# re-ovo/wgpu-path-tracing

Hardware: AMD Instinct MI355X
Metric: Msamples/s (rays x bounces / s) (higher is better)
Workload: dtype f32

## Files before the change

wgpu-path-tracing_amd/csrc/pipeline.hip:

```cpp
#include "pt_device.h"
#include "pt_math.h"

namespace {

constexpr int BLOCK = 256;

PT_DEV void camera_ray(const ptmi_camera &cam, uint32_t x, uint32_t y, uint32_t frame, v3 &org, v3 &dir,
                       uint32_t &rng) {
    rng = rng_seed(x, y, frame);
    float jx = rng_f(rng), jy = rng_f(rng);
    float px = (float)x + jx, py = (float)y + jy;
    float uvx = (px / (float)cam.width) * 2.0f - 1.0f;
    float uvy = (py / (float)cam.height) * 2.0f - 1.0f;
    float th = tan1(cam.fov * 0.5f);
    v3 fw = mk3(cam.forward[0], cam.forward[1], cam.forward[2]);
    v3 rt = mk3(cam.right[0], cam.right[1], cam.right[2]);
    v3 up = mk3(cam.up[0], cam.up[1], cam.up[2]);
    v3 pos = mk3(cam.position[0], cam.position[1], cam.position[2]);
    v3 a = scale3(scale3(scale3(rt, uvx), th), cam.aspect);
    v3 b = scale3(scale3(up, uvy), th);
    dir = normalize3(add3(add3(fw, a), b));
    org = pos;
    if (cam.aperture > 0.0f) {
        v3 focal = madd3(dir, cam.focus_distance, pos);
// ... 39 lines not shown
#define PT_TILE_WORDS 1024
#endif
constexpr int TILE_WORDS = PT_TILE_WORDS;
constexpr int TILE_WAVES = TILE_WORDS / 64;

__global__ __launch_bounds__(TILE_WORDS) void k_tile_sums(const uint32_t *__restrict__ count_ptr,
                                                          const uint64_t *__restrict__ alive,
                                                          const uint64_t *__restrict__ shadow,
                                                          uint32_t *__restrict__ tile_sums,
                                                          uint32_t *__restrict__ shadow_tile_sums,
                                                          unsigned long long *__restrict__ stats, uint32_t bounce) {
    __shared__ uint32_t wsum[TILE_WAVES], wssum[TILE_WAVES];
    const uint32_t count = *count_ptr;
    const uint32_t nwords = (count + 63u) >> 6;
    if (blockIdx.x == 0 && threadIdx.x == 0) {
        atomicAdd(&stats[0], (unsigned long long)count); atomicAdd(&stats[8 + bounce], (unsigned long long)count);
    }
    if (blockIdx.x * TILE_WORDS >= nwords) return;
    const uint32_t w = blockIdx.x * TILE_WORDS + threadIdx.x;
    uint32_t c = 0, sc = 0;
    if (w < nwords) { c = (uint32_t)__popcll(alive[w]); if (shadow) sc = (uint32_t)__popcll(shadow[w]); }
    for (int off = 32; off > 0; off >>= 1) { c += __shfl_down(c, off); sc += __shfl_down(sc, off); }
    if ((threadIdx.x & 63u) == 0u) { wsum[threadIdx.x >> 6] = c; wssum[threadIdx.x >> 6] = sc; }
    __syncthreads();
    if (threadIdx.x == 0) {
        uint32_t t = 0, ts = 0;
        for (int i = 0; i < TILE_WAVES; i++) { t += wsum[i]; ts += wssum[i]; }
        tile_sums[blockIdx.x] = t;
        shadow_tile_sums[blockIdx.x] = ts;
        if (ts) { atomicAdd(&stats[1], (unsigned long long)ts); atomicAdd(&stats[2], (unsigned long long)ts); }
    }
}

PT_DEV void scatter_tile(uint32_t tile, const uint32_t *__restrict__ count_ptr, const uint32_t *__restrict__ queue,
                         const uint64_t *__restrict__ alive, const uint32_t *__restrict__ tile_sums,
                         uint32_t *__restrict__ next_queue, uint32_t *__restrict__ next_count) {
    __shared__ uint32_t wtot[TILE_WAVES];
    __shared__ uint32_t tile_base;
    const uint32_t count = *count_ptr;
    const uint32_t nwords = (count + 63u) >> 6;
    const uint32_t ntiles = (nwords + TILE_WORDS - 1) / TILE_WORDS;
    if (tile >= ntiles) {
        if (ntiles == 0 && tile == 0 && threadIdx.x == 0) *next_count = 0;
        return;
    }
    const uint32_t lane = threadIdx.x & 63u, wave = threadIdx.x >> 6;
    uint32_t pre = 0;
    for (uint32_t t = threadIdx.x; t < tile; t += TILE_WORDS) pre += tile_sums[t];
    for (int off = 32; off > 0; off >>= 1) pre += __shfl_down(pre, off);
    if (lane == 0) wtot[wave] = pre;
    __syncthreads();
    if (threadIdx.x == 0) { uint32_t t = 0; for (int i = 0; i < TILE_WAVES; i++) t += wtot[i]; tile_base = t; }
    __syncthreads();
    const uint32_t base0 = tile_base;
    __syncthreads();
    const uint32_t w = tile * TILE_WORDS + threadIdx.x;
    const uint64_t m = w < nwords ? alive[w] : 0ull;
    const uint32_t c = (uint32_t)__popcll(m);
    uint32_t inc = c;
    for (int off = 1; off < 64; off <<= 1) { uint32_t v = __shfl_up(inc, off); if (lane >= (uint32_t)off) inc += v; }
    if (lane == 63u) wtot[wave] = inc;
    __syncthreads();
    uint32_t wbase = 0;
    for (uint32_t i = 0; i < wave; i++) wbase += wtot[i];
    const uint32_t my_off = base0 + wbase + inc - c;
    if (tile == ntiles - 1 && threadIdx.x == TILE_WORDS - 1) *next_count = my_off + c;
    const uint32_t mlo = (uint32_t)m, mhi = (uint32_t)(m >> 32);
    const uint32_t w0 = tile * TILE_WORDS + wave * 64u;
    for (uint32_t j = 0; j < 64u; j++) {
        const uint32_t jlo = __shfl(mlo, (int)j), jhi = __shfl(mhi, (int)j), jbase = __shfl(my_off, (int)j);
        const uint64_t jm = ((uint64_t)jhi << 32) | jlo;
        if (jm == 0ull) continue;
        if ((jm >> lane) & 1ull) {
            const uint32_t below = (uint32_t)__popcll(jm & ((1ull << lane) - 1ull));
            const uint32_t slot = (w0 + j) * 64u + lane;
            next_queue[jbase + below] = queue ? queue[slot] : slot;
        }
    }
}

__global__ __launch_bounds__(TILE_WORDS) void k_scatter(const uint32_t *__restrict__ count_ptr,
                                                        const uint32_t *__restrict__ queue,
                                                        const uint64_t *__restrict__ alive,
                                                        const uint32_t *__restrict__ tile_sums,
                                                        uint32_t *__restrict__ next_queue,
                                                        uint32_t *__restrict__ next_count) {
    scatter_tile(blockIdx.x, count_ptr, queue, alive, tile_sums, next_queue, next_count);
}
__global__ __launch_bounds__(TILE_WORDS) void k_scatter2(uint32_t tiles, const uint32_t *__restrict__ count_ptr,
                                                         const uint32_t *__restrict__ queue,
                                                         const uint64_t *__restrict__ alive, const uint64_t *__restrict__ shadow,
                                                         const uint32_t *__restrict__ tile_sums, const uint32_t *__restrict__ shadow_sums,
                                                         uint32_t *__restrict__ next_queue, uint32_t *__restrict__ next_count,
                                                         uint32_t *__restrict__ shadow_queue, uint32_t *__restrict__ shadow_count) {
    if (blockIdx.x < tiles) scatter_tile(blockIdx.x, count_ptr, queue, alive, tile_sums, next_queue, next_count);
    else scatter_tile(blockIdx.x - tiles, count_ptr, nullptr, shadow, shadow_sums, shadow_queue, shadow_count);
}

__global__ __launch_bounds__(BLOCK) void k_accumulate(DevBand band, uint32_t frame0, uint32_t n_frames,
                                                      const float *__restrict__ L, uint32_t l_stride, float4 *__restrict__ out) {
    const uint32_t npix = band.rows * band.width;
    for (uint32_t pix = blockIdx.x * BLOCK + threadIdx.x; pix < npix; pix += gridDim.x * BLOCK) {
        const size_t oi = (size_t)band.row_of(pix / band.width) * band.width + pix % band.width;
        float4 acc = out[oi];
        for (uint32_t k = 0; k < n_frames; k++) {
            const size_t li = (size_t)k * npix + pix;
            rgb_sc l;
            if (l_stride == 4u) { const float4 v = reinterpret_cast<const float4 *>(L)[li]; l = rgb_sc{v.x, v.y, v.z}; }
            else l = reinterpret_cast<const rgb_sc *>(L)[li];
            float cx = min1(l.x, 2.5f), cy = min1(l.y, 2.5f), cz = min1(l.z, 2.5f);
            uint32_t frame = frame0 + k;
            if (frame > 0u) {
                float t = 1.0f / (float)(frame + 1u);
                cx = mix1(acc.x, cx, t); cy = mix1(acc.y, cy, t); cz = mix1(acc.z, cz, t);
            }
            acc = make_float4(cx, cy, cz, 0.0f);
        }
        out[oi] = acc;
    }
}

__global__ __launch_bounds__(BLOCK) void k_accumulate_aov(DevBand band, uint32_t frame0, uint32_t n_frames, const float4 *__restrict__ rec,
                                                          const ptmi_triangle *__restrict__ tris, uint32_t n_tris,
                                                          float4 *__restrict__ albedo, float4 *__restrict__ normal, uint2 *__restrict__ ids) {
    const uint32_t npix = band.rows * band.width;
    for (uint32_t pix = blockIdx.x * BLOCK + threadIdx.x; pix < npix; pix += gridDim.x * BLOCK) {
        const size_t oi = (size_t)band.row_of(pix / band.width) * band.width + pix % band.width;
        float4 a = albedo ? albedo[oi] : make_float4(0.0f, 0.0f, 0.0f, 0.0f);
        float4 n = normal ? normal[oi] : make_float4(0.0f, 0.0f, 0.0f, 0.0f);
// ... 136 lines not shown
}

}

void pt_launch_exact_math(hipStream_t s, int which, unsigned long long *out) {
    hipLaunchKernelGGL(k_exact_math, dim3(256 * 16), dim3(256), 0, s, which, out);
}
void pt_launch_raygen(hipStream_t s, int blocks, const ptmi_camera &cam, DevBand band, uint32_t frame0,
                      uint32_t n_frames, DevPaths p, uint32_t *count_out) {
    hipLaunchKernelGGL(k_raygen, dim3(blocks), dim3(BLOCK), 0, s, cam, band, frame0, n_frames, p, count_out);
}
void pt_launch_raygen_list(hipStream_t s, const ptmi_camera &cam, uint32_t n, const uint32_t *xs,
                           const uint32_t *ys, const uint32_t *frames, DevPaths p) {
    hipLaunchKernelGGL(k_raygen_list, dim3((n + BLOCK - 1) / BLOCK), dim3(BLOCK), 0, s, cam, n, xs, ys, frames, p);
}
void pt_launch_compact(hipStream_t s, int tiles, const uint32_t *queue, const uint32_t *count,
                       const uint64_t *alive_mask, const uint64_t *shadow_mask, uint32_t *tile_sums,
                       uint32_t *next_queue, uint32_t *next_count, uint32_t *shadow_queue, uint32_t *shadow_count,
                       unsigned long long *stats, uint32_t bounce, int do_scatter) {
    uint32_t *shadow_sums = tile_sums + tiles;
    hipLaunchKernelGGL(k_tile_sums, dim3(tiles), dim3(TILE_WORDS), 0, s, count, alive_mask, shadow_mask, tile_sums,
                       shadow_sums, stats, bounce);
#ifndef PT_NO_SCATTER2
    if (do_scatter && shadow_mask) {
        hipLaunchKernelGGL(k_scatter2, dim3(2 * tiles), dim3(TILE_WORDS), 0, s, (uint32_t)tiles, count, queue, alive_mask, shadow_mask,
                           tile_sums, shadow_sums, next_queue, next_count, shadow_queue, shadow_count);
        return;
    }
#endif
    if (do_scatter)
        hipLaunchKernelGGL(k_scatter, dim3(tiles), dim3(TILE_WORDS), 0, s, count, queue, alive_mask, tile_sums,
                           next_queue, next_count);
    if (shadow_mask)
        hipLaunchKernelGGL(k_scatter, dim3(tiles), dim3(TILE_WORDS), 0, s, count, (const uint32_t *)nullptr,
                           shadow_mask, shadow_sums, shadow_queue, shadow_count);
}
void pt_launch_accumulate(hipStream_t s, int blocks, DevBand band, uint32_t frame0, uint32_t n_frames,
                          const float *L, uint32_t l_stride, float4 *out) {
    hipLaunchKernelGGL(k_accumulate, dim3(blocks), dim3(BLOCK), 0, s, band, frame0, n_frames, L, l_stride, out);
}
void pt_launch_accumulate_aov(hipStream_t s, int blocks, DevBand band, uint32_t frame0, uint32_t n_frames, const float4 *rec,
                              const ptmi_triangle *tris, uint32_t n_tris, float4 *albedo, float4 *normal, uint2 *ids) {
    hipLaunchKernelGGL(k_accumulate_aov, dim3(blocks), dim3(BLOCK), 0, s, band, frame0, n_frames, rec, tris, n_tris, albedo, normal,
                       ids);
}
void pt_launch_accumulate_moments(hipStream_t s, int blocks, DevBand band, uint32_t frame0, uint32_t n_frames, const float *L,
                                  uint32_t l_stride, float4 *mom) {
    hipLaunchKernelGGL(k_accumulate_moments, dim3(blocks), dim3(BLOCK), 0, s, band, frame0, n_frames, L, l_stride, mom);
}
void pt_launch_pack_rows(hipStream_t s, int blocks, DevBand band, const float4 *frame, float4 *packed) {
    hipLaunchKernelGGL(k_pack_rows, dim3(blocks), dim3(BLOCK), 0, s, band, frame, packed);
}
void pt_launch_unpack_rows(hipStream_t s, int blocks, DevBand band, const float4 *packed, float4 *frame) {
    hipLaunchKernelGGL(k_unpack_rows, dim3(blocks), dim3(BLOCK), 0, s, band, packed, frame);
}
void pt_launch_blit(hipStream_t s, int blocks, uint32_t W, uint32_t H, const float4 *color, float4 *out_f32,
                    uint32_t *out_rgba8) {
    hipLaunchKernelGGL(k_blit, dim3(blocks), dim3(BLOCK), 0, s, W, H, color, out_f32, out_rgba8);
}
void pt_launch_math(hipStream_t s, int op, uint32_t n, const float *a, const float *b, const float *c, float *out) {
    hipLaunchKernelGGL(k_math, dim3((n + 255) / 256), dim3(256), 0, s, op, n, a, b, c, out);
}

uint32_t pt_compact_tile_slots(void) { return TILE_WORDS * 64u; }
```

wgpu-path-tracing_amd/csrc/pt_device.h:

```cpp
#pragma once
#include <hip/hip_runtime.h>
#include <stdint.h>
#include "ptmi_layout.h"

#define PT_HD __host__ __device__ inline

#define PT_REF_LEAF      0x80000000u
#define PT_REF_NONE      0xFFFFFFFFu
#define PT_LEAF_MAX_TRIS 32u
#define PT_LEAF_OFF_BITS 26u
#define PT_LEAF_OFF_MASK ((1u << PT_LEAF_OFF_BITS) - 1u)

struct DevScene;
struct DevScene {
    const ptmi_triangle *tris;  uint32_t n_tris;
    const ptmi_material *mats;  uint32_t n_mats;
    const ptmi_light *lights;   uint32_t n_lights;
    const void *atlas;          uint32_t atlas_w, atlas_h, atlas_fmt;
    const float4 *wnodes;       uint32_t n_wnodes;
    const float4 *tripos;
    float root_min[3], root_max[3];
    uint32_t root_ref;
    const float4 *ref_wnodes;   uint32_t ref_root_ref, has_fast;
    const uint4 *qnodes;        const uint32_t *leaf_stream;
// ... 4 lines not shown
    const float4 *ref_tripos;
    const float4 *tri_leafbox;
    float ref_root_min[3], ref_root_max[3];
    float safe_origin;
    const float4 *wnodes16, *ref_wnodes16;
    uint32_t root_ref16, ref_root_ref16;
    const uint4 *qnodes16;
    unsigned long long *verify_stat;
    const DevScene *self;
};

struct rgb_sc { float x, y, z; };
struct DevPaths {
    float4 *O, *D; float2 *C; float *L; uint32_t l_stride = 3;
    __device__ __forceinline__ rgb_sc ldL(uint32_t p) const {
        if (l_stride == 4u) { const float4 v = reinterpret_cast<const float4 *>(L)[p]; return rgb_sc{v.x, v.y, v.z}; }
        return reinterpret_cast<const rgb_sc *>(L)[p];
    }
    __device__ __forceinline__ void stL(uint32_t p, float x, float y, float z) const {
        if (l_stride == 4u) reinterpret_cast<float4 *>(L)[p] = make_float4(x, y, z, 0.0f);
        else reinterpret_cast<rgb_sc *>(L)[p] = rgb_sc{x, y, z};
    }
};
struct DevShadow { float4 *SO, *SD; rgb_sc *SC; uint32_t cap; };

struct DevBand {
    uint32_t width, height, y0, y1, strip, parts, part, rows;
    PT_HD uint32_t row_of(uint32_t l) const {
        if (parts <= 1u) return y0 + l;
        return y0 + ((l / strip) * parts + part) * strip + l % strip;
    }
};

struct ShadeParams {
    uint32_t bounce, max_bounces, do_mis;
    unsigned long long *stats;
    uint32_t emit_records;
};

enum { PT_VARIANT_GLOBAL = 1, PT_VARIANT_LDS = 2, PT_VARIANT_LDS_NODES = 3,
       PT_VARIANT_OWN_LDS = 4, PT_VARIANT_OWN_LDS_NODES = 5, PT_VARIANT_OWN_QLDS = 6, PT_VARIANT_OWN_QLDS_NODES = 7,
       PT_VARIANT_OWN_QGLOBAL = 8, PT_VARIANT_OWN_GLOBAL = 9,
       PT_VARIANT_OWN_LDS16_NODES = 10,
       PT_VARIANT_OWN_QLDS16_NODES = 11,
       PT_VARIANT_COUNT };

enum PtNodes {
    PT_NODES_EXACT,
    PT_NODES_QUANT,
    PT_NODES_EXACT16,
    PT_NODES_QUANT16 };
enum PtWhere {
    PT_LDS_ALL,
    PT_LDS_NODES,
    PT_FROM_MEMORY };
enum PtStack {
    PT_STACK_DEPTH,
    PT_STACK_NODES,
    PT_STACK_SPILL,
    PT_STACK_16BIT,
    PT_STACK_16BIT_SPILL };
struct PtVariant { PtNodes nodes; PtWhere where; PtStack stack; bool own; };
constexpr PtVariant kPtVariants[PT_VARIANT_COUNT] = {
    {},
    {PT_NODES_EXACT,   PT_FROM_MEMORY, PT_STACK_SPILL,       false},
    {PT_NODES_EXACT,   PT_LDS_ALL,     PT_STACK_DEPTH,       false},
    {PT_NODES_EXACT,   PT_LDS_NODES,   PT_STACK_NODES,       false},
    {PT_NODES_EXACT,   PT_LDS_ALL,     PT_STACK_DEPTH,       true},
    {PT_NODES_EXACT,   PT_LDS_NODES,   PT_STACK_NODES,       true},
    {PT_NODES_QUANT,   PT_LDS_ALL,     PT_STACK_DEPTH,       true},
// ... 22 lines not shown
    int wgs_per_cu;
    size_t lds_bytes;
    uint32_t *spill;
    int wants_spill;
    int quantized;
};
inline uint32_t pt_variant_code(const TraverseConfig &cfg) { return (uint32_t)cfg.variant * 10u + (uint32_t)cfg.wgs_per_cu; }
#ifndef PT_QCACHE_NODES
#define PT_QCACHE_NODES 256
#endif
#define PT_SPILL_ENTRIES 64
size_t pt_spill_bytes(int blocks);

void pt_launch_raygen(hipStream_t s, int blocks, const ptmi_camera &cam, DevBand band, uint32_t frame0,
                      uint32_t n_frames, DevPaths p, uint32_t *count_out);
void pt_launch_raygen_list(hipStream_t s, const ptmi_camera &cam, uint32_t n, const uint32_t *xs,
                           const uint32_t *ys, const uint32_t *frames, DevPaths p);
void pt_launch_extend(hipStream_t s, int blocks, const TraverseConfig &cfg, const DevScene &sc, DevPaths p,
                      const uint32_t *queue, const uint32_t *count, float2 *hits);
void pt_launch_extend_own(hipStream_t s, int blocks, const TraverseConfig &cfg, const DevScene &sc, DevPaths p,
                          const uint32_t *queue, const uint32_t *count, float2 *hits);
void pt_launch_hit_uv(hipStream_t s, uint32_t n, const DevScene &sc, DevPaths p, const float2 *hits, float2 *uv);
void pt_launch_shadow(hipStream_t s, int blocks, const TraverseConfig &cfg, const DevScene &sc, DevPaths p,
                      DevShadow sh, const uint32_t *shadow_queue, const uint32_t *count, uint8_t *occluded_out);
void pt_launch_shadow_own(hipStream_t s, int blocks, const TraverseConfig &cfg, const DevScene &sc, DevPaths p,
                          DevShadow sh, const uint32_t *shadow_queue, const uint32_t *count, uint8_t *occluded_out);
void pt_launch_shade(hipStream_t s, int blocks, const DevScene &sc, DevPaths p, const uint32_t *queue,
                     const uint32_t *count, const float2 *hits, DevShadow sh, uint64_t *alive_mask,
                     uint64_t *shadow_mask, ShadeParams sp, float4 *aov = nullptr);
void pt_launch_shade_fast(hipStream_t s, int blocks, const DevScene &sc, DevPaths p, const uint32_t *queue,
                          const uint32_t *count, const float2 *hits, DevShadow sh, uint64_t *alive_mask,
                          uint64_t *shadow_mask, ShadeParams sp, float4 *aov = nullptr);
uint32_t pt_compact_tile_slots(void);
void pt_launch_compact(hipStream_t s, int tiles, const uint32_t *queue, const uint32_t *count,
                       const uint64_t *alive_mask, const uint64_t *shadow_mask, uint32_t *tile_sums,
                       uint32_t *next_queue, uint32_t *next_count, uint32_t *shadow_queue, uint32_t *shadow_count,
                       unsigned long long *stats, uint32_t bounce, int do_scatter);
void pt_launch_accumulate(hipStream_t s, int blocks, DevBand band, uint32_t frame0, uint32_t n_frames,
                          const float *L, uint32_t l_stride, float4 *out);
void pt_launch_accumulate_aov(hipStream_t s, int blocks, DevBand band, uint32_t frame0, uint32_t n_frames, const float4 *rec,
                              const ptmi_triangle *tris, uint32_t n_tris, float4 *albedo, float4 *normal, uint2 *ids);
void pt_launch_accumulate_moments(hipStream_t s, int blocks, DevBand band, uint32_t frame0, uint32_t n_frames, const float *L,
                                  uint32_t l_stride, float4 *mom);
struct DenoiseArgs {
    uint32_t W, H, iterations;
    float phi_color, phi_normal, phi_depth;
};
void pt_launch_denoise(hipStream_t s, const DenoiseArgs &a, const float4 *radiance, const float4 *normal, const float4 *albedo,
                       const float4 *moments, float4 *guide, float *grad, float4 *cv, float4 *tmp, float4 *out);
void pt_launch_blit(hipStream_t s, int blocks, uint32_t W, uint32_t H, const float4 *color, float4 *out_f32,
                    uint32_t *out_rgba8);
void pt_launch_pack_rows(hipStream_t s, int blocks, DevBand band, const float4 *frame, float4 *packed);
void pt_launch_unpack_rows(hipStream_t s, int blocks, DevBand band, const float4 *packed, float4 *frame);
struct ptmi_options;
DevBand pt_band_of(const ptmi_options &opt, uint32_t width, uint32_t height);
struct ptmi_ctx;
struct PtPrepared;
PtPrepared *pt_prepare_scene(ptmi_ctx *c, const ptmi_triangle *tris, uint32_t nt, const ptmi_material *mats, uint32_t nm,
                             const ptmi_bvh_node *nodes, uint32_t nn, const ptmi_light *lights, uint32_t nl, int *rc_out);
int pt_install_scene(ptmi_ctx *c, PtPrepared *p);
void pt_free_prepared(PtPrepared *p);
int pt_atlas_bytes(uint32_t width, uint32_t height, int format, size_t *bytes, char *why, size_t why_len);
hipStream_t pt_ctx_stream(ptmi_ctx *c);
float4 *pt_ctx_output(ptmi_ctx *c);
int pt_ctx_device(const ptmi_ctx *c);
int pt_ctx_cus(const ptmi_ctx *c);
// ... 4 lines not shown
```

wgpu-path-tracing_amd/csrc/ptmi_api.hip:

```cpp
#include "ptmi.h"
#include "pt_device.h"
#include "fast_tree.h"

#include <algorithm>
#include <chrono>
#include <cmath>
#include <cstdarg>
#include <cstdint>
#include <cstdio>
#include <cstring>
#include <deque>
#include <memory>
#include <string>
#include <typeinfo>
#include <utility>
#include <vector>

namespace {

thread_local std::string g_create_err;

enum SceneBuf {
    kTris, kMats, kLights,
    kRefWnodes, kRefTripos,
    kWnodes, kTripos,
    kQnodes, kLeafStream,
    kLeafbox,
    kWnodes16, kRefWnodes16, kQnodes16,
    kSceneBufs
};

struct EventPair { hipEvent_t a, b; int kind; };
constexpr size_t kMaxPendingEvents = 4096;

}

struct Lane {
    size_t cap = 0;
    DevPaths paths{};
    float2 *hits = nullptr;
    DevShadow sh[2]{};
    uint32_t *queue[2] = {nullptr, nullptr}, *sq[2] = {nullptr, nullptr};
    uint64_t *alive = nullptr, *shadowm = nullptr;
    size_t mask_words = 0;
    uint32_t *word_off = nullptr, *counts = nullptr;
    uint32_t *d_spill = nullptr;
    uint32_t *d_spill_side = nullptr;
    uint8_t *d_occ = nullptr;
    hipStream_t side = nullptr;
    hipEvent_t ev_ready = nullptr, ev_shadow[2] = {nullptr, nullptr};
    float4 *aov = nullptr;
};

struct ptmi_ctx {
    int device = 0, n_cu = 256;
    hipStream_t own_stream = nullptr, stream = nullptr;
    Lane lane;
    mutable std::string err;
    bool alloc_oom = false;
    ptmi_options opt{};

    void *buf[kSceneBufs] = {};
    void *d_atlas = nullptr;
    DevScene *d_scene = nullptr;
    DevScene sc{};
    bool have_scene = false;
    ptmi_image_info img{};

    uint32_t W = 0, H = 0;
    float4 *d_out_own = nullptr, *d_out = nullptr;
    uint32_t aov_mask = 0;
    float4 *d_aov_albedo = nullptr, *d_aov_normal = nullptr;
    uint2 *d_aov_id = nullptr;
    bool moments_on = false;
    float4 *d_moments = nullptr;
// ... 74 lines not shown
constexpr size_t kMaxDispatchesInFlight = 256;

hipError_t throttle(ptmi_ctx *c, size_t max) {
    while (!c->in_flight.empty() && hipEventQuery(c->in_flight.front()) == hipSuccess) {
        c->event_pool.push_back(c->in_flight.front()); c->in_flight.pop_front();
    }
    (void)hipGetLastError();
    while (c->in_flight.size() > max) {
        hipError_t e = hipEventSynchronize(c->in_flight.front());
        if (e != hipSuccess) return e;
        c->event_pool.push_back(c->in_flight.front()); c->in_flight.pop_front();
    }
    return hipSuccess;
}

struct Timed {
    ptmi_ctx *c; hipEvent_t a = nullptr, b = nullptr; int kind; bool on;
    hipStream_t st;
    Timed(ptmi_ctx *c_, int kind_, bool on_, hipStream_t st_ = nullptr) : c(c_), kind(kind_), on(on_), st(st_ ? st_ : c_->stream) {
        if (on) { a = get_event(c); b = get_event(c); (void)hipEventRecord(a, st); }
    }
    ~Timed() {
        if (!on) return;
        (void)hipEventRecord(b, st);
        c->pending.push_back({a, b, kind});
        if (c->pending.size() > kMaxPendingEvents) drain_completed_events(c);
    }
};

void free_batch(Lane &ln) {
    dfree(ln.paths.O); dfree(ln.paths.D); dfree(ln.paths.C); dfree(ln.paths.L);
    dfree(ln.hits);
    for (int k = 0; k < 2; k++) { dfree(ln.sh[k].SO); ln.sh[k].SD = nullptr; ln.sh[k].SC = nullptr; dfree(ln.sq[k]); }
    dfree(ln.queue[0]); dfree(ln.queue[1]); dfree(ln.alive); dfree(ln.shadowm); dfree(ln.word_off); dfree(ln.d_occ);
    dfree(ln.aov);
    ln.cap = 0;
}

hipError_t sync_all(ptmi_ctx *c) {
    hipError_t e = c->stream ? hipStreamSynchronize(c->stream) : hipSuccess;
    if (e == hipSuccess && c->lane.side) e = hipStreamSynchronize(c->lane.side);
    if (e == hipSuccess && c->stream) e = hipStreamSynchronize(c->stream);
    return e;
}

constexpr size_t kBytesPerPath = 16 + 16 + 8 + 16 + 8 + 2 * (16 + 16 + sizeof(rgb_sc) + 4) + 2 * 4 + 1 + 1;
constexpr size_t kAovBytesPerPath = 32;
size_t bytes_per_path(bool aov) { return kBytesPerPath + (aov ? kAovBytesPerPath : 0); }

int ensure_capacity(ptmi_ctx *c, Lane &ln, size_t n) {
    const bool aov = c->aov_mask != 0;
    if (n <= ln.cap && (!aov || ln.aov)) return PTMI_OK;
    HIP_TRY(c, sync_all(c));
    free_batch(ln);
    size_t cap = (n + 1023) & ~(size_t)1023;
    size_t words = cap / 64 + 1;
    size_t tiles = cap / pt_compact_tile_slots() + 2;
    c->alloc_oom = false;
#define ALLOC(ptr, bytes) do { hipError_t e_ = hipMalloc(&(ptr), (bytes)); if (e_ != hipSuccess) { \
        c->alloc_oom = e_ == hipErrorOutOfMemory; free_batch(ln); (void)hipGetLastError(); \
        return fail(c, PTMI_E_HIP, "hipMalloc of %zu bytes for a batch of %zu paths failed: %s", (size_t)(bytes), cap, hipGetErrorString(e_)); } } while (0)
    ALLOC(ln.paths.O, cap * 16); ALLOC(ln.paths.D, cap * 16);
    ALLOC(ln.paths.C, cap * 8); ALLOC(ln.paths.L, cap * 16);
    ALLOC(ln.hits, cap * 8);
    for (int k = 0; k < 2; k++) {
        ALLOC(ln.sh[k].SO, cap * (16 + 16 + sizeof(rgb_sc)));
        ln.sh[k].SD = ln.sh[k].SO + cap; ln.sh[k].SC = reinterpret_cast<rgb_sc *>(ln.sh[k].SO + 2 * cap); ln.sh[k].cap = (uint32_t)cap;
        ALLOC(ln.sq[k], cap * 4);
    }
    ALLOC(ln.queue[0], cap * 4); ALLOC(ln.queue[1], cap * 4);
    ALLOC(ln.alive, words * 8); ALLOC(ln.shadowm, words * 8); ln.mask_words = words;
    ALLOC(ln.word_off, 2 * tiles * 4);
    ALLOC(ln.d_occ, cap);
    if (aov) ALLOC(ln.aov, cap * kAovBytesPerPath);
#undef ALLOC
    ln.cap = cap;
    return PTMI_OK;
}

struct HeldBuf {
    bool present = false;
    std::shared_ptr<const void> keep;
    const std::type_info *type = nullptr;
    const void *host = nullptr;
    void *dev = nullptr;
    int device = -1;
    size_t bytes = 0;
};

struct Built {
    HeldBuf buf[kSceneBufs];
    ptmi_image_info img{};
    uint32_t ref_root_ref = PT_REF_NONE;
    float ref_root_min[3] = {0, 0, 0}, ref_root_max[3] = {0, 0, 0};
    uint32_t root_ref16 = PT_REF_NONE, ref_root_ref16 = PT_REF_NONE;
    uint32_t q_top = 0;
    float tri_safe_dsum = 0.0f;
    uint32_t tree_builder_used = 0;
    double tree_ms = 0.0;

    Built() { img.leaves_used = 1; img.root_ref = PT_REF_NONE; }
    Built(const Built &) = delete;
// ... 732 lines not shown
    const TraverseConfig cfg0 = traverse_config(c, true), cfg_shadow0 = traverse_config(c, false);
    if (c->opt.traversal == PTMI_TRAVERSAL_LDS && pt_variant(cfg0.variant).where != PT_LDS_ALL)
        return fail(c, PTMI_E_UNSUPPORTED, "scene needs %zu B of LDS plus the stack; it does not fit in %zu B", lds_scene_bytes(c), kLdsMax);
    for (;;) {
        rc = ensure_capacity(c, ln, (size_t)(npix * F));
        if (rc == PTMI_OK) break;
        if (!auto_F || !c->alloc_oom || F <= 1) return rc;
        F = (F + 1) / 2;
    }
    if (cfg0.wants_spill && !ln.d_spill) HIP_TRY(c, hipMalloc(&ln.d_spill, pt_spill_bytes(c->n_cu * 8)));
    if (cfg_shadow0.wants_spill && !ln.d_spill_side) HIP_TRY(c, hipMalloc(&ln.d_spill_side, pt_spill_bytes(c->n_cu * 8)));
    c->st.traversal_used = pt_variant(cfg0.variant).where == PT_FROM_MEMORY ? PTMI_TRAVERSAL_GLOBAL : PTMI_TRAVERSAL_LDS;
    c->st.extend_variant = pt_variant_code(cfg0);
    c->st.shadow_variant = pt_variant_code(cfg_shadow0);
    c->st.frames_per_batch_used = F;
    c->st.radiance_stride_bytes = (walks_memory_quantised(cfg0) || walks_memory_quantised(cfg_shadow0)) ? 16u : 12u;
    const int blocks = c->n_cu * 8;
#ifndef PT_SHADE_WGS_PER_CU
#define PT_SHADE_WGS_PER_CU 16
#endif
    const int shade_blocks = c->n_cu * PT_SHADE_WGS_PER_CU;
    const uint32_t maxb = c->opt.max_bounces;
    const bool t1 = c->opt.timing >= 1, t2 = c->opt.timing >= 2, t3 = c->opt.timing >= 3;
    {
        Timed td(c, 0, t1);
        const hipStream_t ms = c->stream;
        const hipStream_t ss = side ? ln.side : ms;
        const int tiles = (int)(ln.cap / pt_compact_tile_slots() + 1);
        TraverseConfig cfg = cfg0, cfg_shadow = cfg_shadow0;
        cfg.spill = ln.d_spill; cfg_shadow.spill = side ? ln.d_spill_side : ln.d_spill;
        if (cfg_shadow.wants_spill && !cfg_shadow.spill) cfg_shadow.spill = ln.d_spill_side;
        ln.paths.l_stride = c->st.radiance_stride_bytes / 4u;
        const DevPaths bp = ln.paths;
        float4 *const aov_rec = c->aov_mask ? ln.aov : nullptr;
        for (uint32_t f0 = 0; f0 < n_frames; f0 += F) {
            const uint32_t fb = std::min(F, n_frames - f0);
            const uint32_t frame0 = cam->frame_index + f0;
            { Timed t(c, 4, t3, ms); pt_launch_raygen(ms, blocks, *cam, band, frame0, fb, bp, &ln.counts[0]); }
            int cur = 0;
            for (uint32_t b = 0; b < maxb; b++) {
                const uint32_t *q = b == 0 ? nullptr : ln.queue[cur];
                const int par = side ? (int)(b & 1u) : 0;
                const ShadeParams shp{b, maxb, c->opt.do_mis, c->d_stats, side ? 1u : 0u};
                { Timed t(c, 1, t2, ms); (c->sc.own ? pt_launch_extend_own : pt_launch_extend)(ms, blocks, cfg, c->sc, bp, q, &ln.counts[b], ln.hits); }
                const bool last = b + 1 == maxb;
                if (side && b >= 2) HIP_TRY(c, hipStreamWaitEvent(ms, ln.ev_shadow[par], 0));
                { Timed t(c, 2, t3, ms);
                  (c->opt.perf_mode ? pt_launch_shade_fast : pt_launch_shade)(
                      ms, shade_blocks, c->sc, bp, q, &ln.counts[b], ln.hits, ln.sh[par], ln.alive, ln.shadowm, shp,
                      b == 0 ? aov_rec : nullptr); }
                { Timed t(c, 5, t3, ms);
                  pt_launch_compact(ms, tiles, q, &ln.counts[b], ln.alive, nee ? ln.shadowm : nullptr,
                                    ln.word_off, ln.queue[cur ^ 1], &ln.counts[b + 1], ln.sq[par], &ln.counts[kShadowCount + par],
                                    c->d_stats, b, last ? 0 : 1); }
                if (side) {
                    HIP_TRY(c, hipEventRecord(ln.ev_ready, ms));
                    HIP_TRY(c, hipStreamWaitEvent(ss, ln.ev_ready, 0));
                    { Timed t(c, 3, t3, ss);
                      (c->sc.own ? pt_launch_shadow_own : pt_launch_shadow)(ss, blocks, cfg_shadow, c->sc, bp, ln.sh[par], ln.sq[par],
                                                                            &ln.counts[kShadowCount + par], nullptr); }
                    HIP_TRY(c, hipEventRecord(ln.ev_shadow[par], ss));
                } else if (nee) {
                    Timed t(c, 3, t3, ms);
                    (c->sc.own ? pt_launch_shadow_own : pt_launch_shadow)(ms, blocks, cfg_shadow, c->sc, bp, ln.sh[0], ln.sq[0], &ln.counts[kShadowCount], nullptr);
                }
                cur ^= 1;
            }
            if (side) {
                HIP_TRY(c, hipStreamWaitEvent(ms, ln.ev_shadow[(maxb - 1) & 1u], 0));
                if (maxb >= 2) HIP_TRY(c, hipStreamWaitEvent(ms, ln.ev_shadow[maxb & 1u], 0));
            }
            { Timed t(c, 6, t3, ms);
              pt_launch_accumulate(ms, blocks, band, frame0, fb, bp.L, bp.l_stride, c->d_out);
              if (aov_rec)
                  pt_launch_accumulate_aov(ms, blocks, band, frame0, fb, aov_rec, c->sc.tris, c->sc.n_tris, c->d_aov_albedo,
                                           c->d_aov_normal, c->d_aov_id);
              if (c->d_moments) pt_launch_accumulate_moments(ms, blocks, band, frame0, fb, bp.L, bp.l_stride, c->d_moments); }
        }
    }
    HIP_TRY(c, hipGetLastError());
    {
        hipEvent_t done = get_event(c);
        HIP_TRY(c, hipEventRecord(done, c->stream));
        c->in_flight.push_back(done);
        if (c->in_flight.size() > kMaxDispatchesInFlight) HIP_TRY(c, throttle(c, kMaxDispatchesInFlight));
    }
    c->st.paths += npix * n_frames;
// ... 492 lines not shown
```

wgpu-path-tracing_amd/csrc/shade.hip:

```cpp
#include "pt_device.h"
#include "pt_math.h"

namespace {

struct HitInfo {
    v3 position; float t;
    v3 normal;
    v3 albedo;
    float roughness, metallic, transmission, ior;
    v3 emission; float emissive_strength;
    bool is_front;
};

PT_DEV v3 ld3(const float *p) { return mk3(p[0], p[1], p[2]); }

PT_DEV v4 atlas_load(const DevScene &sc, uint32_t x, uint32_t y) {
    v4 r; r.x = r.y = r.z = r.w = 0.0f;
    if (sc.atlas_fmt == 0u || x >= sc.atlas_w || y >= sc.atlas_h) return r;
    size_t idx = ((size_t)y * sc.atlas_w + x);
    if (sc.atlas_fmt == 1u) {
        const uint2 raw = reinterpret_cast<const uint2 *>(sc.atlas)[idx];
        union { uint32_t u; _Float16 h[2]; } a, b;
        a.u = raw.x; b.u = raw.y;
        r.x = (float)a.h[0]; r.y = (float)a.h[1]; r.z = (float)b.h[0]; r.w = (float)b.h[1];
// ... 209 lines not shown
        v3 to_l = sub3(lp, hit_pos);
        float dist = length3(to_l);
        v3 wi = vdiv3(to_l, dist);
        v3 e1 = sub3(ld3(T.v1), ld3(T.v0)), e2 = sub3(ld3(T.v2), ld3(T.v0));
        float area = length3(cross3(e1, e2)) * 0.5f;
        float cos_t = __builtin_fabsf(dot3(n, neg3(wi)));
        ls.pdf = (inv_n * rcp1(area)) * (dist * dist / max1(cos_t, PT_EPS));
        ls.intensity = scale3(ld3(lt.color), lt.intensity);
        ls.wi = wi;
        ls.dist = dist;
        ls.traced = true;
    }
    return ls;
}

constexpr int SBLOCK = 256;
#ifndef PT_SHADE_WAVES
#define PT_SHADE_WAVES 0
#endif
#if PT_SHADE_WAVES > 0
#define PT_SHADE_ATTR __attribute__((amdgpu_waves_per_eu(PT_SHADE_WAVES)))
#else
#define PT_SHADE_ATTR
#endif

template <bool AOV>
__global__ __launch_bounds__(SBLOCK) PT_SHADE_ATTR void k_shade(DevScene sc, DevPaths P, const uint32_t *__restrict__ queue,
                                                  const uint32_t *__restrict__ count_ptr,
                                                  const float2 *__restrict__ hits, DevShadow S,
                                                  uint64_t *__restrict__ alive_mask,
                                                  uint64_t *__restrict__ shadow_mask, ShadeParams sp,
                                                  float4 *__restrict__ aov) {
    const uint32_t count = *count_ptr;
    uint32_t n_skipped = 0, n_emitted = 0;
    for (uint32_t base = blockIdx.x * SBLOCK; base < count; base += gridDim.x * SBLOCK) {
        const uint32_t i = base + threadIdx.x;
        bool alive = false, shadow = false, skipped = false, emitted = false;
        if (i < count) {
            const uint32_t q = queue ? queue[i] : i;
            const float2 h2 = ld_stream(&hits[i]);
            if (!(h2.x < 0.0f)) {
                const float4 o4 = ld_stream(&P.O[q]), d4 = ld_stream(&P.D[q]);
                const uint32_t p = q;
                uint32_t rng = __float_as_uint(o4.w);
                const v3 ro = xyz(o4), rd = xyz(d4);
                v3 thr = mk3(1.0f, 1.0f, 1.0f);
                if (sp.bounce != 0u) { const float2 c2 = ld_stream(&P.C[q]); thr = mk3(d4.w, c2.x, c2.y); }
                const HitInfo hit = make_hitinfo(sc, ro, rd, h2.x, __float_as_uint(h2.y));
                if (AOV) {
                    st_stream(&aov[2 * (size_t)i], make_float4(hit.albedo.x, hit.albedo.y, hit.albedo.z, hit.t));
                    st_stream(&aov[2 * (size_t)i + 1], make_float4(hit.normal.x, hit.normal.y, hit.normal.z, h2.y));
                }
                if (hit.emission.x > 0.0f || hit.emission.y > 0.0f || hit.emission.z > 0.0f) {
                    float att = rcp1(1.0f + hit.t * hit.t);
                    float k = hit.emissive_strength;
                    const v3 e = mk3(thr.x * hit.emission.x * k * att, thr.y * hit.emission.y * k * att, thr.z * hit.emission.z * k * att);
                    if (sp.emit_records) {
                        st_stream(&S.SO[i], make_float4(0.0f, 0.0f, 0.0f, -2.0f));
                        st_stream(&S.SD[i], make_float4(0.0f, 0.0f, 0.0f, __uint_as_float(p)));
                        S.SC[i] = rgb_sc{e.x, e.y, e.z};
                        shadow = true; emitted = true;
                    } else {
                        const rgb_sc l = P.ldL(p);
                        P.stL(p, l.x + e.x, l.y + e.y, l.z + e.z);
                    }
                } else {
                    if (sp.do_mis && sc.n_lights > 0u && hit.transmission == 0.0f && hit.is_front) {
                        LightSample ls = sample_light(sc, rng, hit.position);
                        if (ls.pdf > 0.0f) {
                            v3 V = neg3(normalize3(rd));
                            v4 ev = eval_bsdf(hit, hit.normal, V, ls.wi, hit.is_front);
                            float wmis = power_heuristic(1.0f, ls.pdf, 1.0f, ev.w);
                            v3 direct = vdiv3(scale3(mul3(ls.intensity, mk3(ev.x, ev.y, ev.z)), wmis),
                                              max1(ls.pdf, PT_EPS));
                            v3 contrib = mul3(thr, direct);
                            if ((contrib.x != 0.0f) | (contrib.y != 0.0f) | (contrib.z != 0.0f)) {
                                v3 so = madd3(ls.wi, PT_EPS, hit.position);
                                st_stream(&S.SO[i], make_float4(so.x, so.y, so.z, ls.dist));
                                st_stream(&S.SD[i], make_float4(ls.wi.x, ls.wi.y, ls.wi.z, __uint_as_float(p)));
                                S.SC[i] = rgb_sc{contrib.x, contrib.y, contrib.z};
                                shadow = true;
                            } else {
                                skipped = true;
                            }
                        } else if (ls.traced) {
                            skipped = true;
                        }
                    }
                    v3 dir = sample_bsdf(rng, hit, rd, hit.is_front);
                    v4 ev = eval_bsdf(hit, hit.normal, neg3(normalize3(rd)), dir, hit.is_front);
                    if (!(ev.w <= 0.0f)) {
                        v3 no = madd3(dir, PT_EPS, hit.position);
                        v3 nd = normalize3(dir);
                        thr = mul3(thr, vdiv3(mk3(ev.x, ev.y, ev.z), max1(ev.w, PT_EPS)));
                        alive = true;
                        if (sp.bounce > 2u) {
                            float pr = max1(max1(thr.x, thr.y), thr.z);
                            if (rng_f(rng) > pr) alive = false;
                            else thr = vdiv3(thr, pr);
                        }
                        if (alive && sp.bounce + 1u < sp.max_bounces) {
                            st_stream(&P.O[q], make_float4(no.x, no.y, no.z, __uint_as_float(rng)));
                            st_stream(&P.D[q], make_float4(nd.x, nd.y, nd.z, thr.x));
                            st_stream(&P.C[q], make_float2(thr.y, thr.z));
                        }
                    }
                }
            } else if (AOV) {
                st_stream(&aov[2 * (size_t)i], make_float4(0.0f, 0.0f, 0.0f, 0.0f));
                st_stream(&aov[2 * (size_t)i + 1], make_float4(0.0f, 0.0f, 0.0f, __uint_as_float(0xFFFFFFFFu)));
            } else if (sp.bounce != 0u) {
                const float tx = reinterpret_cast<const float *>(&P.D[q])[3];
                const float2 c2 = ld_stream(&P.C[q]);
                if (!(__builtin_isfinite(tx) & __builtin_isfinite(c2.x) & __builtin_isfinite(c2.y))) {
                    const uint32_t p = q;
                    const v3 e = mk3(tx * 0.0f, c2.x * 0.0f, c2.y * 0.0f);
                    if (sp.emit_records) {
                        st_stream(&S.SO[i], make_float4(0.0f, 0.0f, 0.0f, -2.0f));
                        st_stream(&S.SD[i], make_float4(0.0f, 0.0f, 0.0f, __uint_as_float(p)));
                        S.SC[i] = rgb_sc{e.x, e.y, e.z};
                        shadow = true; emitted = true;
                    } else {
                        const rgb_sc l = P.ldL(p);
                        P.stL(p, l.x + e.x, l.y + e.y, l.z + e.z);
                    }
                }
            }
        }
        const uint64_t am = __ballot(alive), sm = __ballot(shadow), zm = __ballot(skipped), em = __ballot(emitted);
        if ((threadIdx.x & 63u) == 0u && i < count) {
            alive_mask[i >> 6] = am;
            shadow_mask[i >> 6] = sm;
            n_skipped += (uint32_t)__popcll(zm);
            n_emitted += (uint32_t)__popcll(em);
        }
    }
    if (n_skipped) atomicAdd(&sp.stats[1], (unsigned long long)n_skipped);
    if (n_emitted) atomicAdd(&sp.stats[3], (unsigned long long)n_emitted);
}

}

#ifdef PT_SHADE_FAST
#define PT_LAUNCH_SHADE pt_launch_shade_fast
#else
#define PT_LAUNCH_SHADE pt_launch_shade
#endif
void PT_LAUNCH_SHADE(hipStream_t s, int blocks, const DevScene &sc, DevPaths p, const uint32_t *queue,
                     const uint32_t *count, const float2 *hits, DevShadow sh, uint64_t *alive_mask,
                     uint64_t *shadow_mask, ShadeParams sp, float4 *aov) {
    if (aov)
        hipLaunchKernelGGL(k_shade<true>, dim3(blocks), dim3(SBLOCK), 0, s, sc, p, queue, count, hits, sh, alive_mask,
                           shadow_mask, sp, aov);
    else
        hipLaunchKernelGGL(k_shade<false>, dim3(blocks), dim3(SBLOCK), 0, s, sc, p, queue, count, hits, sh, alive_mask,
                           shadow_mask, sp, aov);
}

#ifndef PT_SHADE_FAST
namespace {
__global__ void k_hit_uv(uint32_t n, DevScene sc, DevPaths P, const float2 *__restrict__ hits, float2 *__restrict__ uv) {
    const uint32_t i = blockIdx.x * blockDim.x + threadIdx.x;
    if (i >= n) return;
// ... 15 lines not shown
```

Baseline: 11110.

## Repack surviving path state densely at roulette bounce and pack shadow records per wave

After the first Russian-roulette bounce, a new repack kernel copies surviving paths' origin, direction and throughput into a dense tail buffer, along with a pid indirection. Later bounces then read contiguous state instead of gathering through a sparse queue. Shade now writes shadow records compacted within each wave, and a packed scatter variant emits slot indices directly. The aim is better memory coalescing on later bounces, paid for with an extra kernel launch and copy, more memory per path, and a pid lookup when writing radiance.

```diff
diff --git a/wgpu-path-tracing_amd/csrc/pipeline.hip b/wgpu-path-tracing_amd/csrc/pipeline.hip
--- a/wgpu-path-tracing_amd/csrc/pipeline.hip
+++ b/wgpu-path-tracing_amd/csrc/pipeline.hip
@@ -95,6 +95,7 @@
     }
 }
 
+template <bool PACKED>
 PT_DEV void scatter_tile(uint32_t tile, const uint32_t *__restrict__ count_ptr, const uint32_t *__restrict__ queue,
                          const uint64_t *__restrict__ alive, const uint32_t *__restrict__ tile_sums,
                          uint32_t *__restrict__ next_queue, uint32_t *__restrict__ next_count) {
@@ -137,7 +138,7 @@
         if ((jm >> lane) & 1ull) {
             const uint32_t below = (uint32_t)__popcll(jm & ((1ull << lane) - 1ull));
             const uint32_t slot = (w0 + j) * 64u + lane;
-            next_queue[jbase + below] = queue ? queue[slot] : slot;
+            next_queue[jbase + below] = PACKED ? (w0 + j) * 64u + below : queue ? queue[slot] : slot;
         }
     }
 }
@@ -148,7 +149,14 @@
                                                         const uint32_t *__restrict__ tile_sums,
                                                         uint32_t *__restrict__ next_queue,
                                                         uint32_t *__restrict__ next_count) {
-    scatter_tile(blockIdx.x, count_ptr, queue, alive, tile_sums, next_queue, next_count);
+    scatter_tile<false>(blockIdx.x, count_ptr, queue, alive, tile_sums, next_queue, next_count);
+}
+__global__ __launch_bounds__(TILE_WORDS) void k_scatter_packed(const uint32_t *__restrict__ count_ptr,
+                                                               const uint64_t *__restrict__ shadow,
+                                                               const uint32_t *__restrict__ shadow_sums,
+                                                               uint32_t *__restrict__ shadow_queue,
+                                                               uint32_t *__restrict__ shadow_count) {
+    scatter_tile<true>(blockIdx.x, count_ptr, nullptr, shadow, shadow_sums, shadow_queue, shadow_count);
 }
 __global__ __launch_bounds__(TILE_WORDS) void k_scatter2(uint32_t tiles, const uint32_t *__restrict__ count_ptr,
                                                          const uint32_t *__restrict__ queue,
@@ -156,8 +164,20 @@
                                                          const uint32_t *__restrict__ tile_sums, const uint32_t *__restrict__ shadow_sums,
                                                          uint32_t *__restrict__ next_queue, uint32_t *__restrict__ next_count,
                                                          uint32_t *__restrict__ shadow_queue, uint32_t *__restrict__ shadow_count) {
-    if (blockIdx.x < tiles) scatter_tile(blockIdx.x, count_ptr, queue, alive, tile_sums, next_queue, next_count);
-    else scatter_tile(blockIdx.x - tiles, count_ptr, nullptr, shadow, shadow_sums, shadow_queue, shadow_count);
+    if (blockIdx.x < tiles) scatter_tile<false>(blockIdx.x, count_ptr, queue, alive, tile_sums, next_queue, next_count);
+    else scatter_tile<true>(blockIdx.x - tiles, count_ptr, nullptr, shadow, shadow_sums, shadow_queue, shadow_count);
+}
+
+__global__ __launch_bounds__(BLOCK) void k_repack(const uint32_t *__restrict__ count_ptr, const uint32_t *__restrict__ queue,
+                                                  DevPaths from, DevPaths to, uint32_t *__restrict__ pid) {
+    const uint32_t n = *count_ptr;
+    for (uint32_t j = blockIdx.x * BLOCK + threadIdx.x; j < n; j += gridDim.x * BLOCK) {
+        const uint32_t q = queue[j];
+        const float4 o = ld_stream(&from.O[q]), d = ld_stream(&from.D[q]);
+        const float2 c = ld_stream(&from.C[q]);
+        st_stream(&to.O[j], o); st_stream(&to.D[j], d); st_stream(&to.C[j], c);
+        pid[j] = q;
+    }
 }
 
 __global__ __launch_bounds__(BLOCK) void k_accumulate(DevBand band, uint32_t frame0, uint32_t n_frames,
@@ -360,8 +380,12 @@
         hipLaunchKernelGGL(k_scatter, dim3(tiles), dim3(TILE_WORDS), 0, s, count, queue, alive_mask, tile_sums,
                            next_queue, next_count);
     if (shadow_mask)
-        hipLaunchKernelGGL(k_scatter, dim3(tiles), dim3(TILE_WORDS), 0, s, count, (const uint32_t *)nullptr,
-                           shadow_mask, shadow_sums, shadow_queue, shadow_count);
+        hipLaunchKernelGGL(k_scatter_packed, dim3(tiles), dim3(TILE_WORDS), 0, s, count, shadow_mask, shadow_sums, shadow_queue,
+                           shadow_count);
+}
+void pt_launch_repack(hipStream_t s, int blocks, const uint32_t *count, const uint32_t *queue, DevPaths from, DevPaths to,
+                      uint32_t *pid) {
+    hipLaunchKernelGGL(k_repack, dim3(blocks), dim3(BLOCK), 0, s, count, queue, from, to, pid);
 }
 void pt_launch_accumulate(hipStream_t s, int blocks, DevBand band, uint32_t frame0, uint32_t n_frames,
                           const float *L, uint32_t l_stride, float4 *out) {
diff --git a/wgpu-path-tracing_amd/csrc/pt_device.h b/wgpu-path-tracing_amd/csrc/pt_device.h
--- a/wgpu-path-tracing_amd/csrc/pt_device.h
+++ b/wgpu-path-tracing_amd/csrc/pt_device.h
@@ -60,10 +60,14 @@
     }
 };
 
+PT_HD bool pt_plays_roulette(uint32_t bounce) { return bounce > 2u; }
+inline uint32_t pt_repack_bounce() { uint32_t b = 0; while (!pt_plays_roulette(b)) b++; return b; }
+
 struct ShadeParams {
     uint32_t bounce, max_bounces, do_mis;
     unsigned long long *stats;
     uint32_t emit_records;
+    const uint32_t *pid;
 };
 
 enum { PT_VARIANT_GLOBAL = 1, PT_VARIANT_LDS = 2, PT_VARIANT_LDS_NODES = 3,
@@ -152,6 +156,8 @@
                           const uint32_t *count, const float2 *hits, DevShadow sh, uint64_t *alive_mask,
                           uint64_t *shadow_mask, ShadeParams sp, float4 *aov = nullptr);
 uint32_t pt_compact_tile_slots(void);
+void pt_launch_repack(hipStream_t s, int blocks, const uint32_t *count, const uint32_t *queue, DevPaths from, DevPaths to,
+                      uint32_t *pid);
 void pt_launch_compact(hipStream_t s, int tiles, const uint32_t *queue, const uint32_t *count,
                        const uint64_t *alive_mask, const uint64_t *shadow_mask, uint32_t *tile_sums,
                        uint32_t *next_queue, uint32_t *next_count, uint32_t *shadow_queue, uint32_t *shadow_count,
diff --git a/wgpu-path-tracing_amd/csrc/ptmi_api.hip b/wgpu-path-tracing_amd/csrc/ptmi_api.hip
--- a/wgpu-path-tracing_amd/csrc/ptmi_api.hip
+++ b/wgpu-path-tracing_amd/csrc/ptmi_api.hip
@@ -41,6 +41,8 @@
     float2 *hits = nullptr;
     DevShadow sh[2]{};
     uint32_t *queue[2] = {nullptr, nullptr}, *sq[2] = {nullptr, nullptr};
+    DevPaths tail{};
+    uint32_t *pid = nullptr;
     uint64_t *alive = nullptr, *shadowm = nullptr;
     size_t mask_words = 0;
     uint32_t *word_off = nullptr, *counts = nullptr;
@@ -181,6 +183,7 @@
     dfree(ln.paths.O); dfree(ln.paths.D); dfree(ln.paths.C); dfree(ln.paths.L);
     dfree(ln.hits);
     for (int k = 0; k < 2; k++) { dfree(ln.sh[k].SO); ln.sh[k].SD = nullptr; ln.sh[k].SC = nullptr; dfree(ln.sq[k]); }
+    dfree(ln.tail.O); dfree(ln.tail.D); dfree(ln.tail.C); dfree(ln.pid);
     dfree(ln.queue[0]); dfree(ln.queue[1]); dfree(ln.alive); dfree(ln.shadowm); dfree(ln.word_off); dfree(ln.d_occ);
     dfree(ln.aov);
     ln.cap = 0;
@@ -193,7 +196,10 @@
     return e;
 }
 
-constexpr size_t kBytesPerPath = 16 + 16 + 8 + 16 + 8 + 2 * (16 + 16 + sizeof(rgb_sc) + 4) + 2 * 4 + 1 + 1;
+constexpr size_t kBytesPerPath = 16 + 16 + 8 + 16 + 8 + 2 * (16 + 16 + sizeof(rgb_sc) + 4) + (16 + 16 + 8 + 4) + 2 * 4 + 1 + 1;
+#ifndef PT_REPACK
+#define PT_REPACK 1
+#endif
 constexpr size_t kAovBytesPerPath = 32;
 size_t bytes_per_path(bool aov) { return kBytesPerPath + (aov ? kAovBytesPerPath : 0); }
 
@@ -217,6 +223,7 @@
         ln.sh[k].SD = ln.sh[k].SO + cap; ln.sh[k].SC = reinterpret_cast<rgb_sc *>(ln.sh[k].SO + 2 * cap); ln.sh[k].cap = (uint32_t)cap;
         ALLOC(ln.sq[k], cap * 4);
     }
+    ALLOC(ln.tail.O, cap * 16); ALLOC(ln.tail.D, cap * 16); ALLOC(ln.tail.C, cap * 8); ALLOC(ln.pid, cap * 4);
     ALLOC(ln.queue[0], cap * 4); ALLOC(ln.queue[1], cap * 4);
     ALLOC(ln.alive, words * 8); ALLOC(ln.shadowm, words * 8); ln.mask_words = words;
     ALLOC(ln.word_off, 2 * tiles * 4);
@@ -1015,6 +1022,9 @@
         if (cfg_shadow.wants_spill && !cfg_shadow.spill) cfg_shadow.spill = ln.d_spill_side;
         ln.paths.l_stride = c->st.radiance_stride_bytes / 4u;
         const DevPaths bp = ln.paths;
+        const uint32_t rb = PT_REPACK ? pt_repack_bounce() : 0xFFFFFFFEu;
+        DevPaths tp = ln.tail;
+        tp.L = bp.L; tp.l_stride = bp.l_stride;
         float4 *const aov_rec = c->aov_mask ? ln.aov : nullptr;
         for (uint32_t f0 = 0; f0 < n_frames; f0 += F) {
             const uint32_t fb = std::min(F, n_frames - f0);
@@ -1022,20 +1032,23 @@
             { Timed t(c, 4, t3, ms); pt_launch_raygen(ms, blocks, *cam, band, frame0, fb, bp, &ln.counts[0]); }
             int cur = 0;
             for (uint32_t b = 0; b < maxb; b++) {
-                const uint32_t *q = b == 0 ? nullptr : ln.queue[cur];
+                const bool tail = b > rb;
+                const uint32_t *q = b == 0 || b == rb + 1 ? nullptr : ln.queue[cur];
+                const DevPaths sp = tail ? tp : bp;
                 const int par = side ? (int)(b & 1u) : 0;
-                const ShadeParams shp{b, maxb, c->opt.do_mis, c->d_stats, side ? 1u : 0u};
-                { Timed t(c, 1, t2, ms); (c->sc.own ? pt_launch_extend_own : pt_launch_extend)(ms, blocks, cfg, c->sc, bp, q, &ln.counts[b], ln.hits); }
+                const ShadeParams shp{b, maxb, c->opt.do_mis, c->d_stats, side ? 1u : 0u, tail ? ln.pid : nullptr};
+                { Timed t(c, 1, t2, ms); (c->sc.own ? pt_launch_extend_own : pt_launch_extend)(ms, blocks, cfg, c->sc, sp, q, &ln.counts[b], ln.hits); }
                 const bool last = b + 1 == maxb;
                 if (side && b >= 2) HIP_TRY(c, hipStreamWaitEvent(ms, ln.ev_shadow[par], 0));
                 { Timed t(c, 2, t3, ms);
                   (c->opt.perf_mode ? pt_launch_shade_fast : pt_launch_shade)(
-                      ms, shade_blocks, c->sc, bp, q, &ln.counts[b], ln.hits, ln.sh[par], ln.alive, ln.shadowm, shp,
+                      ms, shade_blocks, c->sc, sp, q, &ln.counts[b], ln.hits, ln.sh[par], ln.alive, ln.shadowm, shp,
                       b == 0 ? aov_rec : nullptr); }
                 { Timed t(c, 5, t3, ms);
                   pt_launch_compact(ms, tiles, q, &ln.counts[b], ln.alive, nee ? ln.shadowm : nullptr,
                                     ln.word_off, ln.queue[cur ^ 1], &ln.counts[b + 1], ln.sq[par], &ln.counts[kShadowCount + par],
-                                    c->d_stats, b, last ? 0 : 1); }
+                                    c->d_stats, b, last ? 0 : 1);
+                  if (b == rb && !last) pt_launch_repack(ms, blocks, &ln.counts[b + 1], ln.queue[cur ^ 1], bp, tp, ln.pid); }
                 if (side) {
                     HIP_TRY(c, hipEventRecord(ln.ev_ready, ms));
                     HIP_TRY(c, hipStreamWaitEvent(ss, ln.ev_ready, 0));
diff --git a/wgpu-path-tracing_amd/csrc/shade.hip b/wgpu-path-tracing_amd/csrc/shade.hip
--- a/wgpu-path-tracing_amd/csrc/shade.hip
+++ b/wgpu-path-tracing_amd/csrc/shade.hip
@@ -265,16 +265,19 @@
                                                   uint64_t *__restrict__ shadow_mask, ShadeParams sp,
                                                   float4 *__restrict__ aov) {
     const uint32_t count = *count_ptr;
+    const uint32_t lane = threadIdx.x & 63u;
     uint32_t n_skipped = 0, n_emitted = 0;
     for (uint32_t base = blockIdx.x * SBLOCK; base < count; base += gridDim.x * SBLOCK) {
         const uint32_t i = base + threadIdx.x;
         bool alive = false, shadow = false, skipped = false, emitted = false;
+        float4 rec_o = make_float4(0.0f, 0.0f, 0.0f, -2.0f), rec_d = make_float4(0.0f, 0.0f, 0.0f, 0.0f);
+        rgb_sc rec_c{0.0f, 0.0f, 0.0f};
         if (i < count) {
             const uint32_t q = queue ? queue[i] : i;
             const float2 h2 = ld_stream(&hits[i]);
             if (!(h2.x < 0.0f)) {
                 const float4 o4 = ld_stream(&P.O[q]), d4 = ld_stream(&P.D[q]);
-                const uint32_t p = q;
+                const uint32_t p = sp.pid ? sp.pid[q] : q;
                 uint32_t rng = __float_as_uint(o4.w);
                 const v3 ro = xyz(o4), rd = xyz(d4);
                 v3 thr = mk3(1.0f, 1.0f, 1.0f);
@@ -289,9 +292,8 @@
                     float k = hit.emissive_strength;
                     const v3 e = mk3(thr.x * hit.emission.x * k * att, thr.y * hit.emission.y * k * att, thr.z * hit.emission.z * k * att);
                     if (sp.emit_records) {
-                        st_stream(&S.SO[i], make_float4(0.0f, 0.0f, 0.0f, -2.0f));
-                        st_stream(&S.SD[i], make_float4(0.0f, 0.0f, 0.0f, __uint_as_float(p)));
-                        S.SC[i] = rgb_sc{e.x, e.y, e.z};
+                        rec_d.w = __uint_as_float(p);
+                        rec_c = rgb_sc{e.x, e.y, e.z};
                         shadow = true; emitted = true;
                     } else {
                         const rgb_sc l = P.ldL(p);
@@ -309,9 +311,9 @@
                             v3 contrib = mul3(thr, direct);
                             if ((contrib.x != 0.0f) | (contrib.y != 0.0f) | (contrib.z != 0.0f)) {
                                 v3 so = madd3(ls.wi, PT_EPS, hit.position);
-                                st_stream(&S.SO[i], make_float4(so.x, so.y, so.z, ls.dist));
-                                st_stream(&S.SD[i], make_float4(ls.wi.x, ls.wi.y, ls.wi.z, __uint_as_float(p)));
-                                S.SC[i] = rgb_sc{contrib.x, contrib.y, contrib.z};
+                                rec_o = make_float4(so.x, so.y, so.z, ls.dist);
+                                rec_d = make_float4(ls.wi.x, ls.wi.y, ls.wi.z, __uint_as_float(p));
+                                rec_c = rgb_sc{contrib.x, contrib.y, contrib.z};
                                 shadow = true;
                             } else {
                                 skipped = true;
@@ -327,7 +329,7 @@
                         v3 nd = normalize3(dir);
                         thr = mul3(thr, vdiv3(mk3(ev.x, ev.y, ev.z), max1(ev.w, PT_EPS)));
                         alive = true;
-                        if (sp.bounce > 2u) {
+                        if (pt_plays_roulette(sp.bounce)) {
                             float pr = max1(max1(thr.x, thr.y), thr.z);
                             if (rng_f(rng) > pr) alive = false;
                             else thr = vdiv3(thr, pr);
@@ -346,12 +348,11 @@
                 const float tx = reinterpret_cast<const float *>(&P.D[q])[3];
                 const float2 c2 = ld_stream(&P.C[q]);
                 if (!(__builtin_isfinite(tx) & __builtin_isfinite(c2.x) & __builtin_isfinite(c2.y))) {
-                    const uint32_t p = q;
+                    const uint32_t p = sp.pid ? sp.pid[q] : q;
                     const v3 e = mk3(tx * 0.0f, c2.x * 0.0f, c2.y * 0.0f);
                     if (sp.emit_records) {
-                        st_stream(&S.SO[i], make_float4(0.0f, 0.0f, 0.0f, -2.0f));
-                        st_stream(&S.SD[i], make_float4(0.0f, 0.0f, 0.0f, __uint_as_float(p)));
-                        S.SC[i] = rgb_sc{e.x, e.y, e.z};
+                        rec_d.w = __uint_as_float(p);
+                        rec_c = rgb_sc{e.x, e.y, e.z};
                         shadow = true; emitted = true;
                     } else {
                         const rgb_sc l = P.ldL(p);
@@ -361,7 +362,13 @@
             }
         }
         const uint64_t am = __ballot(alive), sm = __ballot(shadow), zm = __ballot(skipped), em = __ballot(emitted);
-        if ((threadIdx.x & 63u) == 0u && i < count) {
+        if (shadow) {
+            const uint32_t r = (i & ~63u) + (uint32_t)__popcll(sm & ((1ull << lane) - 1ull));
+            st_stream(&S.SO[r], rec_o);
+            st_stream(&S.SD[r], rec_d);
+            S.SC[r] = rec_c;
+        }
+        if (lane == 0u && i < count) {
             alive_mask[i >> 6] = am;
             shadow_mask[i >> 6] = sm;
             n_skipped += (uint32_t)__popcll(zm);
```

Measured after the change: 11310 (median of 6 runs). +1.9%, better.
